# MinaProtocol/snark-challenge-prover-reference

Hardware: AMD Instinct MI355X
Metric: G1 MSM points/sec at 2^20 (MNT4753) (higher is better)
Workload: dtype u32x27 limbs / u64 columns

## Files before the change

snark-challenge-prover-reference_amd/csrc/field_raw_ops.hip.h:

```cpp
#pragma once
#include "fp_inv.hip.h"

namespace mnt753 {

constexpr int FR_OPS = 6;
constexpr int FR_IN_WORDS = FR_OPS * NL;
constexpr int FR_OUT_WORDS = 2 * NL + 1;

enum FieldRawOp : int {
  FR_MUL = 0,
  FR_SQR,
  FR_MUL2,
  FR_MUL3,
  FR_REDUCE2P,
  FR_ADD,
  FR_SUB,
  FR_NEG,
  FR_HALF,
  FR_MUL_SMALL,
  FR_MUL_S,
  FR_SQR_S,
  FR_MUL_S_IP,
  FR_SQR_S_KEEP,
  FR_SUB_RAW,
  FR_ADDSUB_RAW,
  FR_NORM,
  FR_RAW_MAYBE_ZERO,
  FR_IS_ZERO,
  FR_CANON,
  FR_INV,
  FR_FROM_WIRE,
  FR_TO_WIRE,
  FR_NTT2,
  FR_NUM_OPS
};

template <int M>
HD void field_raw_ntt2(Fp<M>& r0, Fp<M>& r1, const Fp<M> x[FR_OPS], uint32_t k) {
  Fp<M> t, lo[2], hi[2];
  for (int b = 0; b < 2; ++b) {
    const Fp<M>& xl = x[2 * b];
    const Fp<M>& xh = x[2 * b + 1];
    if (k & 2u) t = xh;
    else fp_mul_s(t, x[4], xh);
    fp_sub_raw(hi[b], xl, t);
    fp_addsub_raw(lo[b], xl, t, false);
  }
  Fp<M> yl = (k & 1u) ? hi[0] : lo[0], yh = (k & 1u) ? hi[1] : lo[1];
  if ((k >> 2) == 0) { r0 = yl; r1 = yh; return; }
  fp_mul_s(t, x[5], yh);
  fp_sub_raw(yh, yl, t);
  fp_addsub_raw(yl, yl, t, false);
  if ((k >> 2) == 1) { r0 = yl; r1 = yh; return; }
  fp_norm(r0, yl);
  fp_norm(r1, yh);
}

template <int M>
HD void field_raw_op(int op, const uint32_t* in, uint32_t k, uint32_t* out) {
  Fp<M> x[FR_OPS], r0, r1;
  uint32_t flag = 0;
  for (int j = 0; j < FR_OPS; ++j)
    for (int i = 0; i < NL; ++i) x[j].l[i] = in[j * NL + i];
  fp_zero(r0);
  fp_zero(r1);
  switch (op) {
    case FR_MUL: fp_mul(r0, x[0], x[1]); break;
    case FR_SQR: fp_sqr(r0, x[0]); break;
    case FR_MUL2: fp_mul2(r0, x[0], x[1], x[2], x[3]); break;
    case FR_MUL3: fp_mul3(r0, x[0], x[1], x[2], x[3], x[4], x[5]); break;
    case FR_REDUCE2P: fp_reduce2p<M>(r0, x[0].l); break;
    case FR_ADD: fp_add(r0, x[0], x[1]); break;
    case FR_SUB: fp_sub(r0, x[0], x[1]); break;
    case FR_NEG: fp_neg(r0, x[0]); break;
    case FR_HALF: fp_half(r0, x[0]); break;
    case FR_MUL_SMALL: fp_mul_small(r0, x[0], k); break;
    case FR_MUL_S: fp_mul_s(r0, x[0], x[1]); break;
    case FR_SQR_S: fp_sqr_s(r0, x[0]); break;
    case FR_MUL_S_IP: r0 = x[1]; fp_mul_s_ip(r0, x[0]); r1 = x[0]; break;
    case FR_SQR_S_KEEP: fp_sqr_s_keep(r0, x[0]); r1 = x[0]; break;
    case FR_SUB_RAW: fp_sub_raw(r0, x[0], x[1]); break;
    case FR_ADDSUB_RAW: fp_addsub_raw(r0, x[0], x[1], (k & 1u) != 0); break;
    case FR_NORM: fp_norm(r0, x[0]); break;
    case FR_RAW_MAYBE_ZERO: flag = fp_raw_maybe_zero(x[0]) ? 1u : 0u; break;
    case FR_IS_ZERO: flag = fp_is_zero(x[0]) ? 1u : 0u; break;
    case FR_CANON: fp_canon(r0, x[0]); break;
// ... 12 lines not shown
```

snark-challenge-prover-reference_amd/csrc/fp_inv.hip.h:

```cpp
#pragma once
#include "fp753.hip.h"

namespace mnt753 {

struct InvMat { int32_t u, v, q, r; };

HD int32_t inv_divsteps28(int32_t eta, uint32_t f0, uint32_t g0, InvMat& t) {
  uint32_t u = 1, v = 0, q = 0, r = 1;
  uint32_t f = f0, g = g0;
#if defined(__HIP_DEVICE_COMPILE__)
#pragma unroll 4
#endif
  for (int i = 0; i < 28; ++i) {
    uint32_t c1 = (uint32_t)(eta >> 31);
    const uint32_t c2 = 0u - (g & 1u);
    const uint32_t x = (f ^ c1) - c1, y = (u ^ c1) - c1, z = (v ^ c1) - c1;
    g += x & c2; q += y & c2; r += z & c2;
    c1 &= c2;
    eta = (int32_t)(((uint32_t)eta ^ c1) - (c1 + 1u));
    f += g & c1; u += q & c1; v += r & c1;
    g >>= 1; u <<= 1; v <<= 1;
  }
  t.u = (int32_t)u; t.v = (int32_t)v; t.q = (int32_t)q; t.r = (int32_t)r;
  return eta;
// ... 50 lines not shown
#endif
  for (int it = 0; it < 78; ++it) {
    InvMat t;
    eta = inv_divsteps28(eta, (uint32_t)f[0], (uint32_t)g[0], t);
    inv_update_de<M>(d, e, t);
    inv_update_fg(f, g, t);
  }
  const int32_t sf = f[NL - 1] >> 31;
  int32_t c = 0;
#pragma unroll
  for (int i = 0; i < NL; ++i) {
    int32_t v = (d[i] ^ sf) - sf + c;
    if (i < NL - 1) { c = v >> LB; v &= (int32_t)LMASK; }
    d[i] = v;
  }
#pragma unroll 1
  for (int pass = 0; pass < 2; ++pass) {
    const int32_t neg = d[NL - 1] >> 31;
    c = 0;
#pragma unroll
    for (int i = 0; i < NL; ++i) {
      int32_t v = d[i] + ((int32_t)FPC[M].p[i] & neg) + c;
      if (i < NL - 1) { c = v >> LB; v &= (int32_t)LMASK; }
      d[i] = v;
    }
  }
  {
    int32_t s[NL];
    c = 0;
#pragma unroll
    for (int i = 0; i < NL; ++i) {
      int32_t v = d[i] - (int32_t)FPC[M].p[i] + c;
      if (i < NL - 1) { c = v >> LB; v &= (int32_t)LMASK; }
      s[i] = v;
    }
    const int32_t ge = ~(s[NL - 1] >> 31);
#pragma unroll
    for (int i = 0; i < NL; ++i) d[i] = (s[i] & ge) | (d[i] & ~ge);
  }
#pragma unroll
  for (int i = 0; i < NL; ++i) r[i] = (uint32_t)d[i];
}

template <int M>
HD void fp_inv(Fp<M>& r, const Fp<M>& x) {
  Fp<M> c, y, r2, t;
  fp_canon(c, x);
  fp_inv_integer<M>(y.l, c.l);
  fp_const_limbs(r2, FPC[M].r2p);
  fp_mul(t, y, r2);
  fp_mul(r, t, r2);
}

}
```

snark-challenge-prover-reference_amd/csrc/mnt753_testhooks.hip:

```cpp
#include <hip/hip_runtime.h>

#include "common_host.hpp"
#include "../../include/mnt753_hip_test.h"
#include "msm_kernels.hip.h"
#include "field_raw_ops.hip.h"

using namespace mnt753;

namespace {
template <int M>
__global__ void __launch_bounds__(64) k_field_op(int op, const uint32_t* __restrict__ a_wire, const uint32_t* __restrict__ b_wire,
                                                uint32_t* __restrict__ out_wire, size_t n) {
  const size_t i = (size_t)blockIdx.x * blockDim.x + threadIdx.x;
  if (i >= n) return;
  uint32_t wa[24], wb[24], wo[24];
  load_wire24(wa, a_wire + 24 * i);
  load_wire24(wb, b_wire + 24 * i);
  if (op == 4) {
    fp_wire_to_integer<M>(wo, wa);
    store_wire24(out_wire + 24 * i, wo);
    return;
  }
  Fp<M> a, b, r;
  fp_from_wire(a, wa);
  fp_from_wire(b, wb);
  switch (op) {
    case 0: fp_mul(r, a, b); break;
    case 1: fp_add(r, a, b); break;
    case 2: fp_sub(r, a, b); break;
    case 3: fp_inv(r, a); break;
    case 5: fp_neg(r, a); break;
    case 6: fp_sqr(r, a); break;
    case 8: fp_mul2(r, a, b, a, a); break;
    case 9: fp_mul_small(r, a, 13u); break;
    default: r = a; break;
  }
  fp_to_wire(wo, r);
  store_wire24(out_wire + 24 * i, wo);
}
}

extern "C" int mnt753_test_field_op(int mod, int op, const uint64_t* a, const uint64_t* b, size_t n, uint64_t* out) {
  if (mod < 0 || mod > 1 || op < 0 || op > 9 || (n && (!a || !b || !out))) return set_error(MNT753_EINVAL, "test_field_op: bad argument");
  if (int rc = require_device()) return rc;
  if (n == 0) return 0;
  struct Buf {
    uint32_t* p = nullptr;
    ~Buf() { if (p) (void)hipFree(p); }
  } da, db, dout;
  HIP_TRY(hipMalloc(&da.p, 96 * n));
  HIP_TRY(hipMalloc(&db.p, 96 * n));
  HIP_TRY(hipMalloc(&dout.p, 96 * n));
  HIP_TRY(hipMemcpy(da.p, a, 96 * n, hipMemcpyHostToDevice));
  HIP_TRY(hipMemcpy(db.p, b, 96 * n, hipMemcpyHostToDevice));
  const unsigned g = (unsigned)((n + 63) / 64);
  if (mod == MOD_A) hipLaunchKernelGGL((k_field_op<MOD_A>), dim3(g), dim3(64), 0, 0, op, da.p, db.p, dout.p, n);
  else hipLaunchKernelGGL((k_field_op<MOD_B>), dim3(g), dim3(64), 0, 0, op, da.p, db.p, dout.p, n);
  HIP_TRY(hipGetLastError());
  HIP_TRY(hipMemcpy(out, dout.p, 96 * n, hipMemcpyDeviceToHost));
  return 0;
}

namespace {
struct DevBuf {
  uint32_t* p = nullptr;
  ~DevBuf() { if (p) (void)hipFree(p); }
};

template <int M>
__global__ void __launch_bounds__(64) k_field_raw(int op, const uint32_t* __restrict__ in, uint32_t k, uint32_t* __restrict__ out, size_t n) {
  const size_t i = (size_t)blockIdx.x * blockDim.x + threadIdx.x;
  if (i >= n) return;
  field_raw_op<M>(op, in + FR_IN_WORDS * i, k, out + FR_OUT_WORDS * i);
}
}

extern "C" int mnt753_test_field_raw(int mod, int op, const uint32_t* in, size_t n, uint32_t k, uint32_t* out) {
  if (mod < 0 || mod > 1 || op < 0 || op >= FR_NUM_OPS || (n && (!in || !out)) || n > 0x7fffffffu)
    return set_error(MNT753_EINVAL, "test_field_raw: bad argument");
  if (int rc = require_device()) return rc;
  if (n == 0) return 0;
  DevBuf din, dout;
  HIP_TRY(hipMalloc(&din.p, sizeof(uint32_t) * FR_IN_WORDS * n));
  HIP_TRY(hipMalloc(&dout.p, sizeof(uint32_t) * FR_OUT_WORDS * n));
  HIP_TRY(hipMemcpy(din.p, in, sizeof(uint32_t) * FR_IN_WORDS * n, hipMemcpyHostToDevice));
  const unsigned g = (unsigned)((n + 63) / 64);
  if (mod == MOD_A) hipLaunchKernelGGL((k_field_raw<MOD_A>), dim3(g), dim3(64), 0, 0, op, din.p, k, dout.p, n);
  else hipLaunchKernelGGL((k_field_raw<MOD_B>), dim3(g), dim3(64), 0, 0, op, din.p, k, dout.p, n);
  HIP_TRY(hipGetLastError());
  HIP_TRY(hipMemcpy(out, dout.p, sizeof(uint32_t) * FR_OUT_WORDS * n, hipMemcpyDeviceToHost));
  return 0;
}

namespace {
template <class F>
__device__ __forceinline__ void ext_load(typename F::E& r, const uint32_t* wire) {
  uint32_t w[24];
  if constexpr (F::LANES == 1) {
#pragma unroll 1
    for (int k = 0; k < F::DEG; ++k) { load_wire24(w, wire + 24 * k); fp_from_wire(F::comp(r, k), w); }
  } else {
    load_wire24(w, wire + 24 * lane_comp<F>());
    fp_from_wire(r, w);
  }
}
template <class F>
__device__ __forceinline__ void ext_store(uint32_t* wire, const typename F::E& a) {
  uint32_t w[24];
  if constexpr (F::LANES == 1) {
#pragma unroll 1
    for (int k = 0; k < F::DEG; ++k) { fp_to_wire(w, F::comp(a, k)); store_wire24(wire + 24 * k, w); }
  } else {
    fp_to_wire(w, a);
    store_wire24(wire + 24 * lane_comp<F>(), w);
  }
}

template <class F>
__global__ void __launch_bounds__(256, 1) k_ext_op(int op, const uint32_t* __restrict__ a_wire, const uint32_t* __restrict__ b_wire,
                                                  uint32_t* __restrict__ out_wire, uint32_t n) {
  using E = typename F::E;
  const uint32_t t = logical_lane<F>();
  const uint32_t i = t < n ? t : n - 1u;
  constexpr int EWW = 24 * F::DEG;
  E a, b, r;
  ext_load<F>(a, a_wire + (size_t)i * EWW);
  ext_load<F>(b, b_wire + (size_t)i * EWW);
  switch (op) {
    case 0: F::mul(r, a, b); break;
    case 1: F::mul(r, a, a); break;
    case 2:
      if constexpr (has_inv<F>::value) F::inv(r, a); else e_inv(r, a, (F*)nullptr);
      break;
    case 3: F::add(r, a, b); break;
    case 4: F::sub(r, a, b); break;
    case 5: F::neg(r, a); break;
    default: {
      E d;
      F::sub(d, a, b);
      const bool z = F::is_zero(d);
// ... 235 lines not shown
```

snark-challenge-prover-reference_amd/csrc/msm_host.hpp:

```cpp
#pragma once
#include <type_traits>
#include <hip/hip_runtime.h>
#include <algorithm>
#include <atomic>
#include <chrono>
#include <cstdio>
#include <cstdlib>
#include <cstring>
#include <vector>

#include "../../include/mnt753_hip.h"
#include "common_host.hpp"
#include "host_field.hpp"
#include "msm_kernels.hip.h"
#include "msm_knobs.hpp"
#include "msm_limits.hpp"
#include "msm_types.hpp"
#include "msm_sort.hpp"
#include "mnt753_generators.h"

using namespace mnt753;

namespace {

// ... 285 lines not shown
        }
      }
      bind_pair_pool(b);
    }
    if (b->pair_cap >= cap1 && b->pair_buckets >= p.n_buckets) return 0;
    free_pair_ws(b);
    bind_pair_pool(b);
    HIP_TRY(hipMalloc(&b->d_fix, sizeof(uint32_t) * nbA));
    HIP_TRY(hipMalloc(&b->d_gen, sizeof(uint32_t) * aff_words<V>()));
    HIP_TRY(hipMalloc(&b->d_irr_offs[0], sizeof(uint32_t) * (nbA + 1)));
    HIP_TRY(hipMalloc(&b->d_irr_offs[1], sizeof(uint32_t) * (nbA + 1)));
    HIP_TRY(hipMalloc(&b->d_irr_src, sizeof(uint32_t) * (capA / 2 + nbA + 64)));
    HIP_TRY(hipMalloc(&b->d_irr_blocks, sizeof(uint32_t) * (nbA / IRR_BLOCK + 4)));
    uint32_t* wire = nullptr; uint8_t* inf = nullptr;
    const size_t gen_bytes = 192 * (size_t)C::F::DEG;
    const uint64_t* gen_wire = b->curve == MNT753_CURVE_MNT4753 ? (C::F::DEG == 1 ? GEN_MNT4_G1 : GEN_MNT4_G2) : (C::F::DEG == 1 ? GEN_MNT6_G1 : GEN_MNT6_G2);
    HIP_TRY(hipMalloc(&wire, gen_bytes)); HIP_TRY(hipMalloc(&inf, 16));
    HIP_TRY(hipMemcpy(wire, gen_wire, gen_bytes, hipMemcpyHostToDevice));
    hipLaunchKernelGGL((k_bases_to_internal<C>), dim3(1), dim3(256), 0, 0, wire, b->d_gen, inf, (size_t)1);
    HIP_TRY(hipDeviceSynchronize());
    HIP_TRY(hipFree(wire)); HIP_TRY(hipFree(inf));
    b->pair_cap = capA;
    b->pair_buckets = nbA;
    return 0;
  } else {
    (void)b; (void)p; (void)n;
    return 0;
  }
}
template <class C>
MsmPlan plan_for(const mnt753_bases* b, size_t n, const MsmKnobs& knobs) {
  MsmPlan p = make_plan(n, b->pre_c, point_lanes<C>(), knobs);
  p.pair_levels = b->no_pair ? 0 : pair_levels<PointCfg<C>>((uint64_t)p.W * n, b, knobs);
  while (p.pair_levels > 0 && (uint64_t)p.W * n + (uint64_t)p.n_buckets * (((uint64_t)1 << p.pair_levels) - 1) >= 0xfffffff0ull) --p.pair_levels;
  if (point_lanes<C>() == 1 && C::F::DEG == 1 && !pair_row_offsets_fit((uint64_t)p.W * std::max<uint64_t>(b->n, n), row_words<C>() / 4)) p.pair_levels = 0;
  if (p.pair_levels > 0 && pair_cap1(p, n) * (uint64_t)point_lanes<C>() * 7u >= 0xffffff00ull) p.pair_levels = 0;
  p.irr_levels = p.pair_levels > 0 ? irr_levels_for<PointCfg<C>>((uint64_t)p.W * n, p.pair_levels, p.n_buckets, b, knobs) : 0;
  return p;
}
template <class V, bool FIRST, bool LAST, bool IRR>
int launch_pair_level(mnt753_bases* b, hipStream_t st, uint32_t lanes, const uint32_t* d_aff, const uint4* src_planes, size_t src_stride,
                      const uint32_t* offs, uint32_t n_buckets, uint32_t shift, uint32_t* out, size_t out_stride, const uint32_t* irr_src) {
  static std::atomic<uint32_t> lds_set{0};
  const uint32_t dev_bit = 1u << (b->device & 31);
  if (!(lds_set.load(std::memory_order_acquire) & dev_bit)) {
    HIP_TRY(hipFuncSetAttribute(reinterpret_cast<const void*>(&k_pair_level<V, FIRST, LAST, IRR>), hipFuncAttributeMaxDynamicSharedMemorySize, (int)PAIR_LDS_BYTES));
    lds_set.fetch_or(dev_bit, std::memory_order_release);
  }
  hipLaunchKernelGGL((k_pair_level<V, FIRST, LAST, IRR>), dim3(blocks_for<typename V::F>(lanes)), dim3(256), PAIR_LDS_BYTES, st, d_aff, b->d_sorted, src_planes,
                     src_stride, offs, n_buckets, shift, out, b->d_sorted2, reinterpret_cast<uint4*>(out), out_stride,
                     reinterpret_cast<uint4*>(b->d_pair_ws), PAIR_MIN_B, lanes, b->d_gen, b->d_fix, irr_src);
  return 0;
}
template <class V, class C>
int pair_and_accumulate(const MsmPlan& p, size_t n, hipStream_t st, const uint32_t* d_aff, mnt753_bases* b, uint32_t* acc_lanes, uint32_t* acc_T, const uint32_t** acc_offs) {
  if constexpr (V::F::DEG == 1 || V::F::LANES > 1) {
    const int levels = p.pair_levels;
    const uint32_t max_lanes = std::min<uint32_t>(machine_lanes(V::F::LANES), V::F::LANES == 3 ? PAIR_MAX_LANES / 3u : PAIR_MAX_LANES / (uint32_t)V::F::LANES);
    const uint32_t min_B = PAIR_MIN_B;
    if (int rc = ensure_pair_ws<V, C>(b, p, n)) return rc;
    PairPool& pool = pair_pool_of(b);
    if (pool.used) HIP_TRY(hipStreamWaitEvent(st, pool.last_acc, 0));
    HIP_TRY(hipMemsetAsync(b->d_fix, 0, sizeof(uint32_t) * (size_t)p.n_buckets, st));
    uint64_t cap = 2 * pair_cap1(p, n);
    const uint4* src_planes = nullptr;
    size_t src_stride = 0;
    const uint32_t* last_rows = nullptr;
    int irr = p.irr_levels;
    {
      uint64_t c = cap >> levels;
      for (int k = 1; k <= irr; ++k) {
        c = c / 2 + p.n_buckets;
        const uint64_t room = ((levels + k - 1) & 1) ? b->pair_cap / 2 + b->pair_buckets : b->pair_cap;
        if (c > room || c > b->pair_cap / 2 + b->pair_buckets + 64) { irr = k - 1; break; }
      }
    }
    g_last_run.irr_levels = irr;
    for (int l = 1; l <= levels; ++l) {
      cap /= 2;
      const uint32_t lanes = (uint32_t)std::min<uint64_t>(max_lanes, (cap + min_B - 1) / min_B);
      uint32_t* out = b->d_pairpts[(l - 1) & 1];
      const int first = l == 1, last = l == levels && irr == 0;
      const size_t out_stride = blk_quads((cap / 2 + 1) * (uint64_t)V::F::LANES + 64);
      const auto level = first ? (last ? launch_pair_level<V, true, true, false> : launch_pair_level<V, true, false, false>)
                               : (last ? launch_pair_level<V, false, true, false> : launch_pair_level<V, false, false, false>);
      if (int rc = level(b, st, lanes, d_aff, src_planes, src_stride, b->d_offsets, p.n_buckets, (uint32_t)(levels - l), out, out_stride, nullptr)) return rc;
#ifdef MNT753_PAIR_TIMING
      {
        unsigned long long h[8], z[8] = {0, 0, 0, 0, 0, 0, 0, 0};
        (void)hipStreamSynchronize(st);
        (void)hipMemcpyFromSymbol(h, HIP_SYMBOL(g_pair_cycles), sizeof(h));
        (void)hipMemcpyToSymbol(HIP_SYMBOL(g_pair_cycles), z, sizeof(z));
        unsigned int slots = 1;
        (void)hipMemcpyFromSymbol(&slots, HIP_SYMBOL(g_pair_slots), sizeof(slots));
        const double per = (double)h[3] * (slots ? slots : 1);
        if (h[3]) fprintf(stderr, "pair level %d: waves %llu slots/wave %u  ticks/slot: forward %.0f (dma issue %.0f, store %.0f)  backward %.0f (dma issue %.0f, store %.0f)  inversion/wave %.0f\n", l, h[3], slots,
                          (double)h[0] / per, (double)h[4] / per, (double)h[5] / per, (double)h[2] / per, (double)h[6] / per, (double)h[7] / per, (double)h[1] / h[3]);
      }
#endif
      src_planes = reinterpret_cast<const uint4*>(out);
      src_stride = out_stride;
      last_rows = out;
    }
    const uint32_t* offs_acc = b->d_offsets;
    for (int k = 1; k <= irr; ++k) {
      const int l = levels + k;
      const uint32_t* offs_in = offs_acc;
      uint32_t* offs_out = b->d_irr_offs[k & 1];
      const uint32_t n_blocks = (p.n_buckets + IRR_BLOCK - 1) / IRR_BLOCK;
      hipLaunchKernelGGL(k_irr_count, dim3(n_blocks), dim3(IRR_BLOCK), 0, st, offs_in, p.n_buckets, b->d_irr_blocks);
      hipLaunchKernelGGL(k_irr_scan, dim3(1), dim3(1024), 0, st, b->d_irr_blocks, n_blocks);
      hipLaunchKernelGGL(k_irr_fill, dim3(n_blocks), dim3(IRR_BLOCK), 0, st, offs_in, p.n_buckets, b->d_irr_blocks, n_blocks, offs_out, b->d_irr_src);
      cap = cap / 2 + p.n_buckets;
      const uint32_t lanes = (uint32_t)std::min<uint64_t>(max_lanes, (cap + min_B - 1) / min_B);
      uint32_t* out = b->d_pairpts[(l - 1) & 1];
      const size_t out_stride = blk_quads((cap / 2 + 1) * (uint64_t)V::F::LANES + 64);
      const auto level = k == irr ? launch_pair_level<V, false, true, true> : launch_pair_level<V, false, false, true>;
      if (int rc = level(b, st, lanes, d_aff, src_planes, src_stride, offs_out, p.n_buckets, 0u, out, out_stride, b->d_irr_src)) return rc;
      src_planes = reinterpret_cast<const uint4*>(out);
      src_stride = out_stride;
      last_rows = out;
      offs_acc = offs_out;
    }
    const uint32_t* src = last_rows;
    const uint32_t lanes_acc = std::min<uint32_t>(p.n_lanes, machine_lanes(V::F::LANES));
    const uint32_t T2 = (uint32_t)std::max<uint64_t>((cap + lanes_acc - 1) / lanes_acc, 8);
    hipLaunchKernelGGL((k_bucket_accumulate<V, true>), dim3(blocks_for<typename V::F>(lanes_acc)), dim3(256), 0, st, src, b->d_sorted2,
                       offs_acc, p.n_buckets, b->d_buckets, b->d_edges, b->d_edge_bucket, T2, lanes_acc, src_stride);
    if (!pool.last_acc) HIP_TRY(hipEventCreateWithFlags(&pool.last_acc, hipEventDisableTiming));
    HIP_TRY(hipEventRecord(pool.last_acc, st));
    pool.used = true;
    *acc_lanes = lanes_acc;
    *acc_T = T2;
    *acc_offs = offs_acc;
    return 0;
  } else {
    (void)p; (void)n; (void)st; (void)d_aff; (void)b; (void)acc_lanes; (void)acc_T; (void)acc_offs;
    return 0;
  }
}

template <class V, class C>
int point_stages(const MsmPlan& p, size_t n, hipStream_t st, const uint32_t* d_aff, mnt753_bases* b, const MsmKnobs& knobs, uint32_t** result) {
  const int n_pair_levels = p.pair_levels;
  uint32_t acc_lanes = p.n_lanes;
  uint32_t acc_T = p.T;
  const uint32_t* acc_offs = b->d_offsets;
  if (n_pair_levels > 0) {
    if (int rc = pair_and_accumulate<V, C>(p, n, st, d_aff, b, &acc_lanes, &acc_T, &acc_offs)) return rc;
  } else {
    hipLaunchKernelGGL((k_bucket_accumulate<V>), dim3(blocks_for<typename V::F>(p.n_lanes)), dim3(256), 0, st, d_aff, b->d_sorted, b->d_offsets,
                       p.n_buckets, b->d_buckets, b->d_edges, b->d_edge_bucket, p.T, p.n_lanes);
  }
  HIP_TRY(hipEventRecord(b->ev[2], st));
  {
    const uint32_t n_slots = 2 * acc_lanes;
    const unsigned gs = (n_slots + 255) / 256;
    const uint32_t blocked = n_pair_levels > 0 ? 1u : 0u;
    const uint32_t t_arg = n_pair_levels > 0 ? acc_T : p.T;
    const uint32_t* offs = acc_offs;
    HIP_TRY(hipMemsetAsync(b->d_edge_flags, 0, sizeof(uint32_t) * 128, st));
    uint32_t level = 0;
    const uint64_t EDGE_FLOW_NODES = knobs.edge_flow_set ? knobs.edge_flow_nodes
                                     : (C::F::DEG == 1 ? 32768 : (Flow<C>::K3 ? 8192 : 16384));
    uint32_t* counts = b->d_edge_flags + 40;
    uint4* lists[2] = {reinterpret_cast<uint4*>(b->d_edge_tmp), reinterpret_cast<uint4*>(b->d_edge_tmp) + acc_lanes};
    uint32_t parity = 0;
    if (acc_lanes > 1)
      hipLaunchKernelGGL((k_edge_nodes<C>), dim3(gs), dim3(256), 0, st, b->d_edge_bucket, offs, p.n_buckets, t_arg, acc_lanes, blocked, 1u, b->d_edge_flags, 0u, lists[0], counts);
    for (uint64_t stride = 1; stride < acc_lanes; stride *= EDGE_TREE_K, ++level) {
      const uint64_t most = std::min<uint64_t>(acc_lanes, 2 * ((uint64_t)acc_lanes / stride) + 1);
// ... 145 lines not shown
```

snark-challenge-prover-reference_amd/csrc/msm_kernels.hip.h:

```cpp
#pragma once
#include <hip/hip_runtime.h>
#include "curve753.hip.h"

namespace mnt753 {

constexpr int FPS_WORDS = 28;
constexpr uint32_t EDGE_NONE = 0xffffffffu;

template <class C>
constexpr int vm_waves() { return 1; }

template <int M>
__device__ __forceinline__ void fp_load(Fp<M>& r, const uint32_t* p) {
  const uint4* q = reinterpret_cast<const uint4*>(p);
#pragma unroll
  for (int i = 0; i < 7; ++i) {
    uint4 v = q[i];
    r.l[4 * i] = v.x;
    r.l[4 * i + 1] = v.y;
    r.l[4 * i + 2] = v.z;
    if (4 * i + 3 < NL) r.l[4 * i + 3] = v.w;
  }
}
template <int M>
// ... 460 lines not shown
  for (int i = 0; i < NL; ++i) {
    const int32_t yi = subtract ? (int32_t)FPC[M].p2[i] - (int32_t)y.l[i] : (int32_t)y.l[i];
    const int32_t t = (int32_t)a.l[i] + yi + c;
    s[i] = (uint32_t)t & LMASK;
    c = t >> LB;
  }
  fp_reduce2p<M>(r, s);
}

__host__ __device__ __forceinline__ size_t blk_index(uint32_t j) { return (size_t)(j >> 6) * (7 * 64) + (j & 63u); }
__host__ __device__ __forceinline__ size_t blk_quads(uint64_t n_elems) { return (size_t)((n_elems + 63) / 64) * (7 * 64); }
template <int M>
__device__ __forceinline__ uint32_t fp_load_blk(Fp<M>& r, const uint4* __restrict__ base, uint32_t j) {
  const uint4* q = base + blk_index(j);
  uint32_t flag = 0;
#pragma unroll
  for (int i = 0; i < 7; ++i) {
    const uint4 v = q[(size_t)i * 64];
    r.l[4 * i] = v.x;
    r.l[4 * i + 1] = v.y;
    r.l[4 * i + 2] = v.z;
    if (4 * i + 3 < NL) r.l[4 * i + 3] = v.w; else flag = v.w;
  }
  return flag;
}
template <int M>
__device__ __forceinline__ void fp_store_blk(uint4* __restrict__ base, uint32_t j, const Fp<M>& a, uint32_t flag) {
  uint4* q = base + blk_index(j);
#pragma unroll
  for (int i = 0; i < 7; ++i) {
    uint4 v;
    v.x = a.l[4 * i];
    v.y = a.l[4 * i + 1];
    v.z = a.l[4 * i + 2];
    v.w = (4 * i + 3 < NL) ? a.l[4 * i + 3] : flag;
    q[(size_t)i * 64] = v;
  }
}

constexpr uint32_t PAIR_IMG_QUADS = 1792;
constexpr uint32_t PAIR_LDS_WAVE_QUADS = PAIR_IMG_QUADS + 448 + 128;
constexpr uint32_t PAIR_LDS_BYTES = 4 * PAIR_LDS_WAVE_QUADS * 16;
#ifndef MNT753_PAIR_DMA_FIRST
#define MNT753_PAIR_DMA_FIRST 4
#endif
#ifndef MNT753_PAIR_DMA_LATER
#define MNT753_PAIR_DMA_LATER 2
#endif
#ifndef MNT753_PAIR_DMA_IRR
#define MNT753_PAIR_DMA_IRR 3
#endif
constexpr uint32_t PAIR_DMA_STEPS_FIRST = MNT753_PAIR_DMA_FIRST, PAIR_DMA_STEPS_LATER = MNT753_PAIR_DMA_LATER, PAIR_DMA_STEPS_IRR = MNT753_PAIR_DMA_IRR;

#ifdef MNT753_PAIR_TIMING
__device__ unsigned long long g_pair_cycles[8];
__device__ unsigned int g_pair_slots;
#define PAIR_T(var) const unsigned long long var = __builtin_readcyclecounter()
#define PAIR_ACC(i, a, b) do { if ((threadIdx.x & 63u) == 0) atomicAdd(&g_pair_cycles[i], (unsigned long long)((b) - (a))); } while (0)
#define PAIR_TW_DECL(var) unsigned long long var = 0
#define PAIR_TW(var, ...) do { const unsigned long long t_a = __builtin_readcyclecounter(); __VA_ARGS__; var += __builtin_readcyclecounter() - t_a; } while (0)
#else
#define PAIR_T(var)
#define PAIR_ACC(i, a, b)
#define PAIR_TW_DECL(var)
#define PAIR_TW(var, ...) do { __VA_ARGS__; } while (0)
#endif
typedef __attribute__((address_space(3))) void* lds_ptr_t;
__device__ __forceinline__ void glds16(const void* gsrc, const uint4* lds_dst_wave_uniform) {
  __builtin_amdgcn_global_load_lds(gsrc, (lds_ptr_t)lds_dst_wave_uniform, 16, 0, 0);
}
__device__ __forceinline__ void glds4(const void* gsrc, const uint32_t* lds_dst_wave_uniform) {
  __builtin_amdgcn_global_load_lds(gsrc, (lds_ptr_t)lds_dst_wave_uniform, 4, 0, 0);
}
__device__ __forceinline__ void wait_vm0() { __builtin_amdgcn_s_waitcnt(0x0f70); asm volatile("" ::: "memory"); }
__device__ __forceinline__ void wait_lgkm0() { __builtin_amdgcn_s_waitcnt(0xc07f); asm volatile("" ::: "memory"); }
template <int M>
__device__ __forceinline__ uint32_t fp_from_lds(Fp<M>& r, const uint4* p, uint32_t stride) {
  uint32_t flag = 0;
#pragma unroll
  for (int i = 0; i < 7; ++i) {
    const uint4 v = p[(size_t)i * stride];
    r.l[4 * i] = v.x;
    r.l[4 * i + 1] = v.y;
    r.l[4 * i + 2] = v.z;
    if (4 * i + 3 < NL) r.l[4 * i + 3] = v.w; else flag = v.w;
  }
  return flag;
}

constexpr uint32_t IRR_BLOCK = 256;
static __global__ void __launch_bounds__(IRR_BLOCK) k_irr_count(const uint32_t* __restrict__ offs_in, uint32_t n_buckets, uint32_t* __restrict__ block_sums) {
  __shared__ uint32_t part[IRR_BLOCK / 64];
  const uint32_t b = blockIdx.x * IRR_BLOCK + threadIdx.x;
  uint32_t c = b < n_buckets ? (offs_in[b + 1] - offs_in[b] + 1u) >> 1 : 0u;
#pragma unroll
  for (int d = 32; d >= 1; d >>= 1) c += __shfl_xor(c, d, 64);
  if ((threadIdx.x & 63u) == 0) part[threadIdx.x >> 6] = c;
  __syncthreads();
  if (threadIdx.x == 0) block_sums[blockIdx.x] = part[0] + part[1] + part[2] + part[3];
}
static __global__ void __launch_bounds__(1024) k_irr_scan(uint32_t* __restrict__ block_sums, uint32_t n_blocks) {
  __shared__ uint32_t wsum[16];
  __shared__ uint32_t carry;
  if (threadIdx.x == 0) carry = 0;
  __syncthreads();
  for (uint32_t base = 0; base < n_blocks; base += 1024) {
// ... 214 lines not shown
        for (uint32_t k = 0; k < ROW_PIECES_X; ++k) glds16(table + off[k], im + 64u * k);
      } else {
        issue_rows(it + AH, (it + AH) & 3u, std::true_type{}, im, sw_nxt);
      }
    };
    if (ahead) issue_ahead(off);
    if constexpr (IRR) { if (it + 2u < n_it) sw_nn = irr_word(it + 2u); }
    uint32_t kind;
    if (!on || (f0 & PF_EMPTY)) kind = PK_EMPTY;
    else if (f1 & PF_EMPTY) kind = PK_SINGLE;
    else {
      kind = PK_ADD;
      bool same_x;
      if constexpr (LAZY) {
        F::sub_raw(den, x2, x1);
        same_x = F::raw_maybe_zero(den);
        if (same_x) { E du; F::sub(du, x2, x1); same_x = F::is_zero(du); }
      } else {
        F::sub(den, x2, x1);
        same_x = F::is_zero(den);
      }
      if (same_x) {
        if constexpr (first) {
          const uint2 e = reinterpret_cast<const uint2*>(entries)[o];
          fp_load(y1, src_rows + (size_t)PAIR_ROW(e.x & 0x7fffffffu) * TW + TY + cw);
          fp_load(y2, src_rows + (size_t)PAIR_ROW(e.y & 0x7fffffffu) * TW + TY + cw);
        } else if constexpr (IRR) {
          const uint32_t s1 = sw_cur & 0x7fffffffu, s2 = s1 + 1u;
          (void)fp_load_blk(y1, src_planes + (2 + (s1 & 1u)) * src_stride, (s1 >> 1) * LN + comp);
          (void)fp_load_blk(y2, src_planes + (2 + (s2 & 1u)) * src_stride, (s2 >> 1) * LN + comp);
        } else {
          (void)fp_load_blk(y1, src_planes + 2 * src_stride, o * LN + comp);
          (void)fp_load_blk(y2, src_planes + 3 * src_stride, o * LN + comp);
        }
        fp_addsub<M>(den, y1, y2, ((f0 ^ f1) & PF_NEG) != 0);
        if (F::is_zero(den)) { F::one(den); kind = PK_CANCEL; } else kind = PK_DBL;
      }
    }
    PAIR_TW(tw_b, if (on) fp_store_blk(prefix_ws, o * LN + comp, run, kind));
    PAIR_T(tfa0);
    asm volatile("" ::: "memory");
#ifdef MNT753_PAIR_TIMING
    tw_a += __builtin_readcyclecounter() - tfa0;
#endif
    if (kind <= PK_CANCEL) {
      if constexpr (LAZY) F::mul_s(tmp, run, den); else F::mul(tmp, run, den);
      run = tmp;
    }
    if constexpr (IRR) { sw_cur = sw_nxt; sw_nxt = sw_nn; }
  }
  E inv;
  PAIR_T(tc1);
  if constexpr (LAZY) { F::norm(tmp, run); run = tmp; }
  F::inv(inv, run);
  PAIR_T(tc2);
  constexpr uint32_t BWD_PIECES = ROW_PIECES + 7u;
  auto issue_bwd_piece = [=](uint32_t it, uint32_t buf, uint32_t idx, uint32_t sw = 0u) __attribute__((always_inline)) {
    if (idx < ROW_PIECES) issue_row_piece(it, buf, idx, std::false_type{}, img, sw);
    else if (idx < BWD_PIECES) {
      const uint32_t o = min(it * NLe + (lane_on ? t : t0w), S - 1u);
      const uint32_t q = idx - ROW_PIECES;
      glds16(prefix_ws + blk_index(o * LN + comp) + (size_t)q * 64, pre_img + q * 64u);
    }
  };
  auto issue_bwd = [=](uint32_t it, uint32_t buf, uint32_t sw = 0u) __attribute__((always_inline)) {
    for (uint32_t idx = 0; idx < BWD_PIECES; ++idx) issue_bwd_piece(it, buf, idx, sw);
  };
  wait_vm0();
  if constexpr (first) {
    issue_entries(n_it - 1u, 0);
    wait_vm0();
    issue_entries(n_it > 1u ? n_it - 2u : 0u, 1);
  }
  if constexpr (IRR) { sw_cur = irr_word(n_it - 1u); sw_nxt = irr_word(n_it > 1u ? n_it - 2u : 0u); }
  issue_bwd(n_it - 1u, 0, sw_cur);
  wait_vm0();
  for (uint32_t n = 0; n < n_it; ++n) {
    const uint32_t it = n_it - 1u - n;
    const uint32_t o = it * NLe + t;
    const bool on = lane_on && o < S;
    uint32_t f0, f1;
    E pre;
    uint32_t sw_nn = 0u;
    if constexpr (IRR) { if (it >= 2u) sw_nn = irr_word(it - 2u); }
    read_rows(n & 1u, std::false_type{}, img, f0, f1, x1, y1, x2, y2);
    if constexpr (IRR) { if (sw_cur >> 31) f1 = PF_EMPTY; }
    uint32_t kflag;
    kflag = fp_from_lds(pre, pre_img + lane, 64u);
    const uint32_t kind = on ? kflag : (uint32_t)PK_EMPTY;
    const bool more = n + 1u < n_it;
    const uint32_t vb_next = more ? (uint32_t)blk_index(min((it - 1u) * NLe + (lane_on ? t : t0w), S - 1u) * LN + comp) : 0u;
    uint32_t va_irr = 0u, vb_irr = 0u;
    if constexpr (IRR) { if (more) irr_bases(sw_nxt, va_irr, vb_irr); }
    wait_lgkm0();
    if constexpr (first) { if (more) issue_entries(it >= 2u ? it - 2u : 0u, n & 1u); }
    const bool flip = ((f0 ^ f1) & PF_NEG) != 0;
    uint32_t out_flag = PF_EMPTY;
    E num, ysave, yo;
    if constexpr (!DIET) {
      ysave = y1;
      if (kind == PK_ADD) {
        out_flag = f1 & PF_NEG;
        if constexpr (LAZY) {
          F::sub_raw(den, x2, x1);
          F::addsub_raw(num, y2, y1, !flip);
        } else {
          F::sub(den, x2, x1);
// ... 664 lines not shown
```

Baseline: 48.39 million.

## Split pair-level field inversion across lane groups with Montgomery batching

In the non-first pair levels with LN==1, each lane's independent field inversion is replaced. The new path multiplies values pairwise across lanes in a butterfly tree (Montgomery batch trick), so a 16-lane group shares one inversion. That inversion is computed cooperatively, with the divstep d/e/f/g limbs spread across the 16 lanes and carries exchanged by DPP shuffles. The aim is to cut the serial per-lane 78-iteration safegcd cost, in exchange for extra multiplies, cross-lane shuffles and zero-handling. A test hook and a refactored timing report are added alongside.

After: 49.20 million (median of 6 runs). 1.7% higher.

```diff
diff --git a/snark-challenge-prover-reference_amd/csrc/field_raw_ops.hip.h b/snark-challenge-prover-reference_amd/csrc/field_raw_ops.hip.h
--- a/snark-challenge-prover-reference_amd/csrc/field_raw_ops.hip.h
+++ b/snark-challenge-prover-reference_amd/csrc/field_raw_ops.hip.h
@@ -6,6 +6,7 @@
 constexpr int FR_OPS = 6;
 constexpr int FR_IN_WORDS = FR_OPS * NL;
 constexpr int FR_OUT_WORDS = 2 * NL + 1;
+constexpr int FR_INV_GROUP_LANES = 16;
 
 enum FieldRawOp : int {
   FR_MUL = 0,
@@ -32,6 +33,7 @@
   FR_FROM_WIRE,
   FR_TO_WIRE,
   FR_NTT2,
+  FR_INV_GROUP = 24,
   FR_NUM_OPS
 };
 
diff --git a/snark-challenge-prover-reference_amd/csrc/fp_inv.hip.h b/snark-challenge-prover-reference_amd/csrc/fp_inv.hip.h
--- a/snark-challenge-prover-reference_amd/csrc/fp_inv.hip.h
+++ b/snark-challenge-prover-reference_amd/csrc/fp_inv.hip.h
@@ -126,4 +126,205 @@
   fp_mul(r, t, r2);
 }
 
-}
+
+template <int G>
+struct InvGrp {
+  static_assert(G == 8 || G == 16 || G == 32, "group sizes: 8, 16 or 32 lanes");
+  static constexpr int LPL = 32 / G;
+  static constexpr int TOP_LANE = (NL - 1) / LPL, TOP_SLOT = (NL - 1) % LPL;
+};
+
+template <int LPL>
+HD void inv_grp_take(int32_t out[LPL], const uint32_t a[NL], int j) {
+#pragma unroll
+  for (int k = 0; k < LPL; ++k) out[k] = 0;
+#pragma unroll
+  for (int i = 0; i < NL; ++i)
+    if (i / LPL == j) out[i % LPL] = (int32_t)a[i];
+}
+template <int LPL>
+HD void inv_grp_masks(uint32_t keep[LPL], int j) {
+#pragma unroll
+  for (int k = 0; k < LPL; ++k) keep[k] = LPL * j + k == NL - 1 ? 0xffffffffu : LMASK;
+}
+template <int LPL, bool WITH_P>
+HD void inv_grp_columns(int32_t lo[LPL], int32_t hi[LPL], const int32_t a[LPL], const int32_t b[LPL], int32_t m0, int32_t m1,
+                        const int32_t pl[LPL], int32_t mp) {
+#pragma unroll
+  for (int k = 0; k < LPL; ++k) {
+    int64_t c = (int64_t)m0 * a[k] + (int64_t)m1 * b[k];
+    if (WITH_P) c += (int64_t)pl[k] * mp;
+    lo[k] = (int32_t)((uint32_t)c & LMASK);
+    hi[k] = (int32_t)(c >> LB);
+  }
+}
+template <int LPL>
+HD void inv_grp_shift(int32_t v[LPL], const int32_t lo[LPL], const int32_t hi[LPL], int32_t lo_next) {
+#pragma unroll
+  for (int k = 0; k < LPL; ++k) v[k] = (k + 1 < LPL ? lo[k + 1] : lo_next) + hi[k];
+}
+HD int32_t inv_grp_carry(int32_t v, uint32_t keep) { return (int32_t)((uint32_t)v & ~keep) >> LB; }
+template <int LPL>
+HD void inv_grp_settle(int32_t out[LPL], const int32_t v[LPL], const uint32_t keep[LPL], int32_t carry_in) {
+#pragma unroll
+  for (int k = 0; k < LPL; ++k) out[k] = (int32_t)((uint32_t)v[k] & keep[k]) + (k ? inv_grp_carry(v[k - 1], keep[k - 1]) : carry_in);
+}
+template <int M>
+HD void inv_grp_pmult(int32_t& md, int32_t& me, const InvMat& t, int32_t sd, int32_t se, uint32_t d0, uint32_t e0) {
+  const uint32_t pinv = (0u - FPC[M].inv) & LMASK;
+  md = (t.u & sd) + (t.v & se);
+  me = (t.q & sd) + (t.r & se);
+  const uint32_t cd = (uint32_t)t.u * d0 + (uint32_t)t.v * e0;
+  const uint32_t ce = (uint32_t)t.q * d0 + (uint32_t)t.r * e0;
+  md -= (int32_t)((pinv * cd + (uint32_t)md) & LMASK);
+  me -= (int32_t)((pinv * ce + (uint32_t)me) & LMASK);
+}
+template <int M>
+HD void inv_grp_finish(uint32_t r[NL], int32_t d[NL], uint32_t f0) {
+  int32_t c;
+#pragma unroll 1
+  for (int pass = 0; pass < 4; ++pass) {
+    const int32_t neg = pass == 0 ? 0 : d[NL - 1] >> 31;
+    c = 0;
+#pragma unroll
+    for (int i = 0; i < NL; ++i) {
+      int32_t v = d[i] + ((int32_t)FPC[M].p[i] & neg) + c;
+      if (i < NL - 1) { c = v >> LB; v &= (int32_t)LMASK; }
+      d[i] = v;
+    }
+  }
+  int32_t s[NL], n[NL];
+  c = 0;
+  int32_t cn = 0, nz = 0;
+#pragma unroll
+  for (int i = 0; i < NL; ++i) {
+    int32_t v = d[i] - (int32_t)FPC[M].p[i] + c;
+    int32_t w = (int32_t)FPC[M].p[i] - d[i] + cn;
+    if (i < NL - 1) { c = v >> LB; v &= (int32_t)LMASK; cn = w >> LB; w &= (int32_t)LMASK; }
+    s[i] = v; n[i] = w;
+    nz |= d[i];
+  }
+  const int32_t ge = ~(s[NL - 1] >> 31);
+  const int32_t sf = f0 == LMASK ? -1 : 0;
+  int32_t ns[NL];
+  cn = 0;
+  int32_t nzs = 0;
+#pragma unroll
+  for (int i = 0; i < NL; ++i) {
+    int32_t w = (int32_t)FPC[M].p[i] - s[i] + cn;
+    if (i < NL - 1) { cn = w >> LB; w &= (int32_t)LMASK; }
+    ns[i] = w;
+    nzs |= s[i];
+  }
+  const int32_t e_nz = (ge ? nzs : nz) != 0 ? -1 : 0;
+#pragma unroll
+  for (int i = 0; i < NL; ++i) {
+    const int32_t e = (s[i] & ge) | (d[i] & ~ge);
+    const int32_t ne = ((ns[i] & ge) | (n[i] & ~ge)) & e_nz;
+    r[i] = (uint32_t)((ne & sf) | (e & ~sf));
+  }
+}
+
+#if defined(__HIPCC__)
+template <int G> __device__ __forceinline__ int32_t inv_grp_from_next(int32_t x) {
+  if constexpr (G == 16) return __builtin_amdgcn_update_dpp(0, x, 0x101, 0xf, 0xf, true);
+  else { const int l = (int)(threadIdx.x & 63u); const int y = __builtin_amdgcn_ds_bpermute(((l + 1) & 63) << 2, x); return (l & (G - 1)) == G - 1 ? 0 : y; }
+}
+template <int G> __device__ __forceinline__ int32_t inv_grp_from_prev(int32_t x) {
+  if constexpr (G == 16) return __builtin_amdgcn_update_dpp(0, x, 0x111, 0xf, 0xf, true);
+  else { const int l = (int)(threadIdx.x & 63u); const int y = __builtin_amdgcn_ds_bpermute(((l - 1) & 63) << 2, x); return (l & (G - 1)) == 0 ? 0 : y; }
+}
+template <int G, int SRC> __device__ __forceinline__ int32_t inv_grp_bcast(int32_t x) {
+  if constexpr (G == 16) return __builtin_amdgcn_update_dpp(0, x, 0x150 + SRC, 0xf, 0xf, false);
+  else { const int l = (int)(threadIdx.x & 63u); return __builtin_amdgcn_ds_bpermute(((l & ~(G - 1)) + SRC) << 2, x); }
+}
+
+template <int G, int I>
+struct InvGrpGather {
+  static __device__ __forceinline__ void run(int32_t D[NL], const int32_t d[InvGrp<G>::LPL]) {
+    D[I] = inv_grp_bcast<G, I / InvGrp<G>::LPL>(d[I % InvGrp<G>::LPL]);
+    if constexpr (I + 1 < NL) InvGrpGather<G, I + 1>::run(D, d);
+  }
+};
+
+template <int M, int G>
+__device__ __forceinline__ void fp_inv_integer_group(uint32_t r[NL], const uint32_t a[NL]) {
+  constexpr int LPL = InvGrp<G>::LPL;
+  const int j = (int)(threadIdx.x & (unsigned)(G - 1));
+  int32_t d[LPL], e[LPL], f[LPL], g[LPL], pl[LPL];
+  uint32_t keep[LPL];
+  inv_grp_take<LPL>(pl, FPC[M].p, j);
+  inv_grp_take<LPL>(g, a, j);
+  inv_grp_masks<LPL>(keep, j);
+#pragma unroll
+  for (int k = 0; k < LPL; ++k) { d[k] = 0; e[k] = 0; f[k] = pl[k]; }
+  if (j == 0) e[0] = 1;
+  int32_t eta = -1;
+#pragma unroll 1
+  for (int it = 0; it < 78; ++it) {
+    InvMat t;
+    const uint32_t f0 = (uint32_t)inv_grp_bcast<G, 0>(f[0]), g0 = (uint32_t)inv_grp_bcast<G, 0>(g[0]);
+    const uint32_t d0 = (uint32_t)inv_grp_bcast<G, 0>(d[0]), e0 = (uint32_t)inv_grp_bcast<G, 0>(e[0]);
+    const int32_t sd = inv_grp_bcast<G, InvGrp<G>::TOP_LANE>(d[InvGrp<G>::TOP_SLOT]) >> 31;
+    const int32_t se = inv_grp_bcast<G, InvGrp<G>::TOP_LANE>(e[InvGrp<G>::TOP_SLOT]) >> 31;
+    eta = inv_divsteps28(eta, f0, g0, t);
+    int32_t md, me;
+    inv_grp_pmult<M>(md, me, t, sd, se, d0, e0);
+    int32_t lo[LPL], hi[LPL], v[4][LPL];
+    inv_grp_columns<LPL, true>(lo, hi, d, e, t.u, t.v, pl, md);
+    inv_grp_shift<LPL>(v[0], lo, hi, inv_grp_from_next<G>(lo[0]));
+    inv_grp_columns<LPL, true>(lo, hi, d, e, t.q, t.r, pl, me);
+    inv_grp_shift<LPL>(v[1], lo, hi, inv_grp_from_next<G>(lo[0]));
+    inv_grp_columns<LPL, false>(lo, hi, f, g, t.u, t.v, pl, 0);
+    inv_grp_shift<LPL>(v[2], lo, hi, inv_grp_from_next<G>(lo[0]));
+    inv_grp_columns<LPL, false>(lo, hi, f, g, t.q, t.r, pl, 0);
+    inv_grp_shift<LPL>(v[3], lo, hi, inv_grp_from_next<G>(lo[0]));
+    inv_grp_settle<LPL>(d, v[0], keep, inv_grp_from_prev<G>(inv_grp_carry(v[0][LPL - 1], keep[LPL - 1])));
+    inv_grp_settle<LPL>(e, v[1], keep, inv_grp_from_prev<G>(inv_grp_carry(v[1][LPL - 1], keep[LPL - 1])));
+    inv_grp_settle<LPL>(f, v[2], keep, inv_grp_from_prev<G>(inv_grp_carry(v[2][LPL - 1], keep[LPL - 1])));
+    inv_grp_settle<LPL>(g, v[3], keep, inv_grp_from_prev<G>(inv_grp_carry(v[3][LPL - 1], keep[LPL - 1])));
+  }
+  int32_t D[NL];
+  InvGrpGather<G, 0>::run(D, d);
+  inv_grp_finish<M>(r, D, (uint32_t)inv_grp_bcast<G, 0>(f[0]));
+}
+
+template <int M, int G>
+__device__ __forceinline__ void fp_inv_group(Fp<M>& r, const Fp<M>& x) {
+  Fp<M> c, y, r2, t;
+  fp_canon(c, x);
+  fp_inv_integer_group<M, G>(y.l, c.l);
+  fp_const_limbs(r2, FPC[M].r2p);
+  fp_mul(t, y, r2);
+  fp_mul(r, t, r2);
+}
+template <int M, int G, int S>
+struct InvLanesLevel {
+  static __device__ __forceinline__ void run(Fp<M>& P) {
+    if constexpr ((1 << S) == G) {
+      const Fp<M> x = P;
+      fp_inv_group<M, G>(P, x);
+    } else {
+      const int src4 = (int)(((threadIdx.x & 63u) ^ (1u << S)) << 2);
+      Fp<M> sib, up;
+#pragma unroll
+      for (int i = 0; i < NL; ++i) sib.l[i] = (uint32_t)__builtin_amdgcn_ds_bpermute(src4, (int)P.l[i]);
+      fp_mul(up, P, sib);
+      InvLanesLevel<M, G, S + 1>::run(up);
+      fp_mul(P, up, sib);
+    }
+  }
+};
+template <int M, int G>
+__device__ __forceinline__ void fp_inv_lanes(Fp<M>& r, const Fp<M>& x) {
+  const bool zero = fp_is_zero(x);
+  Fp<M> P;
+#pragma unroll
+  for (int i = 0; i < NL; ++i) P.l[i] = zero ? FPC[M].one[i] : x.l[i];
+  InvLanesLevel<M, G, 0>::run(P);
+#pragma unroll
+  for (int i = 0; i < NL; ++i) r.l[i] = zero ? 0u : P.l[i];
+}
+#endif
+
+}
diff --git a/snark-challenge-prover-reference_amd/csrc/mnt753_testhooks.hip b/snark-challenge-prover-reference_amd/csrc/mnt753_testhooks.hip
--- a/snark-challenge-prover-reference_amd/csrc/mnt753_testhooks.hip
+++ b/snark-challenge-prover-reference_amd/csrc/mnt753_testhooks.hip
@@ -73,6 +73,33 @@
   if (i >= n) return;
   field_raw_op<M>(op, in + FR_IN_WORDS * i, k, out + FR_OUT_WORDS * i);
 }
+template <int M>
+__global__ void __launch_bounds__(64) k_field_raw_inv_group(const uint32_t* __restrict__ in, uint32_t k, uint32_t* __restrict__ out, size_t n) {
+  constexpr int G = FR_INV_GROUP_LANES;
+  const size_t i = (size_t)blockIdx.x * blockDim.x + threadIdx.x;
+  const uint32_t* rec = in + FR_IN_WORDS * (i < n ? i : n - 1);
+  Fp<M> x, r;
+  for (int l = 0; l < NL; ++l) x.l[l] = rec[l];
+  if (k == 0) {
+    fp_inv_lanes<M, G>(r, x);
+  } else {
+    fp_zero(r);
+    const int lane = (int)(threadIdx.x & 63u);
+#pragma unroll 1
+    for (int s = 0; s < G; ++s) {
+      Fp<M> xs, t;
+      const int src4 = ((lane & ~(G - 1)) + s) << 2;
+#pragma unroll
+      for (int l = 0; l < NL; ++l) xs.l[l] = (uint32_t)__builtin_amdgcn_ds_bpermute(src4, (int)x.l[l]);
+      fp_inv_group<M, G>(t, xs);
+      if ((lane & (G - 1)) == s) r = t;
+    }
+  }
+  if (i >= n) return;
+  uint32_t* o = out + FR_OUT_WORDS * i;
+  for (int l = 0; l < NL; ++l) { o[l] = r.l[l]; o[NL + l] = 0; }
+  o[2 * NL] = 0;
+}
 }
 
 extern "C" int mnt753_test_field_raw(int mod, int op, const uint32_t* in, size_t n, uint32_t k, uint32_t* out) {
@@ -85,7 +112,11 @@
   HIP_TRY(hipMalloc(&dout.p, sizeof(uint32_t) * FR_OUT_WORDS * n));
   HIP_TRY(hipMemcpy(din.p, in, sizeof(uint32_t) * FR_IN_WORDS * n, hipMemcpyHostToDevice));
   const unsigned g = (unsigned)((n + 63) / 64);
-  if (mod == MOD_A) hipLaunchKernelGGL((k_field_raw<MOD_A>), dim3(g), dim3(64), 0, 0, op, din.p, k, dout.p, n);
+  if (op == FR_INV_GROUP) {
+    if (k > 1) return set_error(MNT753_EINVAL, "test_field_raw: FR_INV_GROUP takes k = 0 or 1");
+    if (mod == MOD_A) hipLaunchKernelGGL((k_field_raw_inv_group<MOD_A>), dim3(g), dim3(64), 0, 0, din.p, k, dout.p, n);
+    else hipLaunchKernelGGL((k_field_raw_inv_group<MOD_B>), dim3(g), dim3(64), 0, 0, din.p, k, dout.p, n);
+  } else if (mod == MOD_A) hipLaunchKernelGGL((k_field_raw<MOD_A>), dim3(g), dim3(64), 0, 0, op, din.p, k, dout.p, n);
   else hipLaunchKernelGGL((k_field_raw<MOD_B>), dim3(g), dim3(64), 0, 0, op, din.p, k, dout.p, n);
   HIP_TRY(hipGetLastError());
   HIP_TRY(hipMemcpy(out, dout.p, sizeof(uint32_t) * FR_OUT_WORDS * n, hipMemcpyDeviceToHost));
diff --git a/snark-challenge-prover-reference_amd/csrc/msm_host.hpp b/snark-challenge-prover-reference_amd/csrc/msm_host.hpp
--- a/snark-challenge-prover-reference_amd/csrc/msm_host.hpp
+++ b/snark-challenge-prover-reference_amd/csrc/msm_host.hpp
@@ -361,6 +361,20 @@
                      reinterpret_cast<uint4*>(b->d_pair_ws), PAIR_MIN_B, lanes, b->d_gen, b->d_fix, irr_src);
   return 0;
 }
+#ifdef MNT753_PAIR_TIMING
+static void pair_timing_report(hipStream_t st, int l) {
+  unsigned long long h[8], z[8] = {0, 0, 0, 0, 0, 0, 0, 0};
+  (void)hipStreamSynchronize(st);
+  (void)hipMemcpyFromSymbol(h, HIP_SYMBOL(g_pair_cycles), sizeof(h));
+  (void)hipMemcpyToSymbol(HIP_SYMBOL(g_pair_cycles), z, sizeof(z));
+  unsigned int slots = 1;
+  (void)hipMemcpyFromSymbol(&slots, HIP_SYMBOL(g_pair_slots), sizeof(slots));
+  const double per = (double)h[3] * (slots ? slots : 1);
+  if (h[3]) fprintf(stderr, "pair level %d: waves %llu slots/wave %u  ticks/slot: forward %.0f (dma issue %.0f, store %.0f)  backward %.0f (dma issue %.0f, store %.0f)  inversion/wave %.0f  share %.4f\n", l, h[3], slots,
+                    (double)h[0] / per, (double)h[4] / per, (double)h[5] / per, (double)h[2] / per, (double)h[6] / per, (double)h[7] / per, (double)h[1] / h[3],
+                    (double)h[1] / (double)(h[0] + h[1] + h[2]));
+}
+#endif
 template <class V, class C>
 int pair_and_accumulate(const MsmPlan& p, size_t n, hipStream_t st, const uint32_t* d_aff, mnt753_bases* b, uint32_t* acc_lanes, uint32_t* acc_T, const uint32_t** acc_offs) {
   if constexpr (V::F::DEG == 1 || V::F::LANES > 1) {
@@ -395,17 +409,7 @@
                                : (last ? launch_pair_level<V, false, true, false> : launch_pair_level<V, false, false, false>);
       if (int rc = level(b, st, lanes, d_aff, src_planes, src_stride, b->d_offsets, p.n_buckets, (uint32_t)(levels - l), out, out_stride, nullptr)) return rc;
 #ifdef MNT753_PAIR_TIMING
-      {
-        unsigned long long h[8], z[8] = {0, 0, 0, 0, 0, 0, 0, 0};
-        (void)hipStreamSynchronize(st);
-        (void)hipMemcpyFromSymbol(h, HIP_SYMBOL(g_pair_cycles), sizeof(h));
-        (void)hipMemcpyToSymbol(HIP_SYMBOL(g_pair_cycles), z, sizeof(z));
-        unsigned int slots = 1;
-        (void)hipMemcpyFromSymbol(&slots, HIP_SYMBOL(g_pair_slots), sizeof(slots));
-        const double per = (double)h[3] * (slots ? slots : 1);
-        if (h[3]) fprintf(stderr, "pair level %d: waves %llu slots/wave %u  ticks/slot: forward %.0f (dma issue %.0f, store %.0f)  backward %.0f (dma issue %.0f, store %.0f)  inversion/wave %.0f\n", l, h[3], slots,
-                          (double)h[0] / per, (double)h[4] / per, (double)h[5] / per, (double)h[2] / per, (double)h[6] / per, (double)h[7] / per, (double)h[1] / h[3]);
-      }
+      pair_timing_report(st, l);
 #endif
       src_planes = reinterpret_cast<const uint4*>(out);
       src_stride = out_stride;
@@ -426,6 +430,9 @@
       const size_t out_stride = blk_quads((cap / 2 + 1) * (uint64_t)V::F::LANES + 64);
       const auto level = k == irr ? launch_pair_level<V, false, true, true> : launch_pair_level<V, false, false, true>;
       if (int rc = level(b, st, lanes, d_aff, src_planes, src_stride, offs_out, p.n_buckets, 0u, out, out_stride, b->d_irr_src)) return rc;
+#ifdef MNT753_PAIR_TIMING
+      pair_timing_report(st, l);
+#endif
       src_planes = reinterpret_cast<const uint4*>(out);
       src_stride = out_stride;
       last_rows = out;
diff --git a/snark-challenge-prover-reference_amd/csrc/msm_kernels.hip.h b/snark-challenge-prover-reference_amd/csrc/msm_kernels.hip.h
--- a/snark-challenge-prover-reference_amd/csrc/msm_kernels.hip.h
+++ b/snark-challenge-prover-reference_amd/csrc/msm_kernels.hip.h
@@ -536,6 +536,9 @@
 #endif
 constexpr uint32_t PAIR_DMA_STEPS_FIRST = MNT753_PAIR_DMA_FIRST, PAIR_DMA_STEPS_LATER = MNT753_PAIR_DMA_LATER, PAIR_DMA_STEPS_IRR = MNT753_PAIR_DMA_IRR;
 
+#ifndef MNT753_PAIR_INV_GROUP
+#define MNT753_PAIR_INV_GROUP 16
+#endif
 #ifdef MNT753_PAIR_TIMING
 __device__ unsigned long long g_pair_cycles[8];
 __device__ unsigned int g_pair_slots;
@@ -856,7 +859,8 @@
   E inv;
   PAIR_T(tc1);
   if constexpr (LAZY) { F::norm(tmp, run); run = tmp; }
-  F::inv(inv, run);
+  if constexpr (LN == 1 && !first && MNT753_PAIR_INV_GROUP != 0) fp_inv_lanes<M, MNT753_PAIR_INV_GROUP>(inv, run);
+  else F::inv(inv, run);
   PAIR_T(tc2);
   constexpr uint32_t BWD_PIECES = ROW_PIECES + 7u;
   auto issue_bwd_piece = [=](uint32_t it, uint32_t buf, uint32_t idx, uint32_t sw = 0u) __attribute__((always_inline)) {
```
